# google-research/sparf

Hardware: NVIDIA H100
Metric: rays/sec (fwd+bwd, 128 samples/ray) (higher is better)
Workload: dtype fp32 in / out; GEMMs on Hopper wgmma with a 3-pass error-compensated split (fp16 halves forward, bf16 halves backward), fp32 accumulation; fp32 CUDA cores for encoding / activations / compositing

## Files before the change

### sparf_b200/csrc/gemm_wgmma.cu

```cuda
#include <cuda_bf16.h>
#include <cudaTypedefs.h>
#include <cuda_fp16.h>

#include <algorithm>
#include <type_traits>

#include "gemm_wgmma.cuh"

namespace sparf {
namespace {

constexpr int TM = 128, TN = 128, TK = 32;
constexpr int TILE_ELEMS = TM * TK;

struct __align__(128) WgSmem {
  uint16_t a[2][TILE_ELEMS];
  uint16_t b[2][TILE_ELEMS];
};

__device__ __forceinline__ int sw_off(int r, int k) { return (((r >> 3) * (TK / 8) + (k >> 3)) << 6) + ((r & 7) << 3) + (k & 7); }

__device__ __forceinline__ uint64_t smem_desc(const void* p) {
  uint32_t a = static_cast<uint32_t>(__cvta_generic_to_shared(p));
  uint64_t d = (uint64_t)((a & 0x3FFFF) >> 4);
// ... 777 lines not shown
      mbar_wait(&empty[s], ((it / NST) & 1) ^ 1);
      uint8_t* st = smem + s * STAGE_BYTES;
      if (x.div == 1) {
        if (lane == 0) {
          mbar_expect_tx(&full[s], abytes + TK * TM * 4);
          bulk_g2s(st, a.tile(by, kt0 + j), abytes, &full[s]);
          tensor_g2s(st + 2 * TILE_BYTES, xmap, k0, m0, &full[s]);
        }
        continue;
      }
      if (lane == 0) {
        mbar_expect_tx(&full[s], abytes + min(TK, x.M - m0) * rbytes);
        bulk_g2s(st, a.tile(by, kt0 + j), abytes, &full[s]);
      }
      __syncwarp();
      const int m = m0 + lane;
      if (m < x.M) bulk_g2s(st + 2 * TILE_BYTES + lane * (TM * 4), x.X + (size_t)(m / x.div) * x.ldx + k0, rbytes, &full[s]);
    }
  }
}

template <int PASSES, int NST = STAGES>
__device__ __forceinline__ void convert_staged(const Staged& x, const Units& w, uint64_t* full, uint64_t* conv) {
  extern __shared__ __align__(1024) uint8_t smem[];
  const int t = threadIdx.x - CONSUMERS, lane = t & 31;
  int it = 0;
  for (int u = blockIdx.x; u < w.tiles * w.nsplit; u += gridDim.x) {
    int bx, by, kt0, nk;
    w.get(u, bx, by, kt0, nk);
    const bool kin = bx * TM + t < x.K, bits = x.bits && by == 0;
    const int bword = bx * (TM / 32) + (t >> 5);
    for (int j = 0; j < nk; ++j, ++it) {
      const int s = it % NST, m0 = (kt0 + j) * TK;
      mbar_wait(&full[s], (it / NST) & 1);
      uint8_t* st = smem + s * STAGE_BYTES + 2 * TILE_BYTES;
      const float* src = reinterpret_cast<const float*>(st);
      float v[TK];
      if (kin && m0 + TK <= x.M) {
#pragma unroll
        for (int r = 0; r < TK; ++r) v[r] = src[r * TM + t];
      } else {
#pragma unroll
        for (int r = 0; r < TK; ++r) v[r] = kin && m0 + r < x.M ? src[r * TM + t] : 0.f;
      }
      if (bits) {
        uint32_t word = 0;
#pragma unroll
        for (int r = 0; r < TK; ++r) {
          const uint32_t b = __ballot_sync(0xffffffffu, v[r] > 0.f);
          if (lane == r) word = b;
        }
        if (m0 + lane < x.M && bword < x.kw) x.bits[(size_t)(m0 + lane) * x.kw + bword] = word;
      }
      converter_sync();
      uint16_t* img = reinterpret_cast<uint16_t*>(st);
#pragma unroll
      for (int o = 0; o < TK / 8; ++o) {
        float e8[8];
#pragma unroll
        for (int e = 0; e < 8; ++e) e8[e] = v[8 * o + e];
        uint4 hi, lo;
        split8_mul(e8, hi, lo);
        const int off = sw_off(t, 8 * o);
        *reinterpret_cast<uint4*>(img + off) = hi;
        if (PASSES == 3) *reinterpret_cast<uint4*>(img + TILE_ELEMS + off) = lo;
      }
      fence_proxy_async();
      __syncwarp();
      if (lane == 0) mbar_arrive(&conv[s]);
    }
  }
}

__device__ __forceinline__ int part_off(int r, int c) { return r * TN + (((c >> 3) ^ (r & 7)) << 3) + (c & 7); }

__device__ __forceinline__ void presum_epilogue(const float (&acc)[64], float* part, bool first, bool flush, int bx, int by,
                                                const Epi& e) {
  const int lane = threadIdx.x & 31, w = threadIdx.x >> 5;
#pragma unroll
  for (int i = 0; i < 64; i += 2) {
    float2* p = reinterpret_cast<float2*>(part + part_off(frag_row(i), frag_col(i)));
    if (first) {
      *p = make_float2(acc[i], acc[i + 1]);
    } else {
      const float2 o = *p;
      *p = make_float2(o.x + acc[i], o.y + acc[i + 1]);
    }
  }
  if (!flush) return;
  __syncwarp();
  const int m0 = by * TM, n0 = bx * TN;
  float* out = e.out + e.col_off + n0;
  for (int i = 0; i < 16; ++i) {
    const int r = 16 * w + i, m = m0 + r;
    if (m >= e.M) continue;
#pragma unroll
    for (int q = 0; q < TN / 32; ++q) {
      const int c = 32 * q + lane, n = n0 + c;
      if (n < e.N && n < e.Kv) atomicAdd(out + (size_t)m * e.ldo + c, part[part_off(r, c)]);
    }
  }
  __syncwarp();
}

template <int PASSES, bool DYN = false>
__global__ void __launch_bounds__(STAGED_THREADS, 1) wg_gemm_staged_kernel(Opnd a, Staged x, Units w, Epi e, RowCount rc,
                                                                           int ctas, const __grid_constant__ CUtensorMap xmap) {
  extern __shared__ __align__(1024) uint8_t smem[];
  if constexpr (DYN) {
    x.M = (int)live_rows<true, false>(x.M, rc);
    if (x.M == 0) return;
    w.nk = (x.M + TK - 1) / TK;
    w.nsplit = max(1, min(w.nk, (ctas + w.tiles - 1) / w.tiles * ((w.nk + 1023) / 1024)));
  }
  float* part = reinterpret_cast<float*>(smem + STAGED_STAGES * STAGE_BYTES);
  uint64_t* full = reinterpret_cast<uint64_t*>(smem + STAGED_STAGES * STAGE_BYTES + PART_BYTES);
  uint64_t* empty = full + STAGED_STAGES;
  uint64_t* conv = empty + STAGED_STAGES;
  if (threadIdx.x == 0) {
    for (int i = 0; i < STAGED_STAGES; ++i) {
      mbar_init(&full[i], 1);
      mbar_init(&empty[i], CONSUMERS / 32);
      mbar_init(&conv[i], 4);
    }
    asm volatile("fence.mbarrier_init.release.cluster;\n" ::: "memory");
  }
  __syncthreads();
  if (threadIdx.x >= CONSUMERS + 128) {
    asm volatile("setmaxnreg.dec.sync.aligned.u32 40;\n" ::: "memory");
    if (threadIdx.x < CONSUMERS + 128 + 32) produce_staged<PASSES, STAGED_STAGES>(a, x, &xmap, w, full, empty);
    return;
  }
  if (threadIdx.x >= CONSUMERS) {
    asm volatile("setmaxnreg.dec.sync.aligned.u32 64;\n" ::: "memory");
    convert_staged<PASSES, STAGED_STAGES>(x, w, full, conv);
    return;
  }
  asm volatile("setmaxnreg.inc.sync.aligned.u32 200;\n" ::: "memory");
  const int units = w.tiles * w.nsplit, grid = gridDim.x;
  int it = 0;
  for (int u = blockIdx.x; u < units; u += grid) {
    int bx, by, kt0, nk;
    w.get(u, bx, by, kt0, nk);
    float acc[64];
    mma_unit<false, PASSES, true, STAGED_STAGES>(acc, nk, it, full, empty, conv);
    const int t = u % w.tiles;
    const bool first = u < grid || (u - grid) % w.tiles != t;
    const bool flush = u + grid >= units || (u + grid) % w.tiles != t;
    presum_epilogue(acc, part, first, flush, bx, by, e);
  }
}

constexpr int CH_W = 256;
constexpr int CH_M = 64;
constexpr int CH_KS = CH_W / TK;
constexpr int CH_ENC_KS = 2;
constexpr int CH_HALF = CH_M * TK * 2;
constexpr int CH_STAGES = 4;
constexpr int CH_ENC = CH_KS * 2 * CH_HALF;
constexpr int CH_RING = CH_ENC + CH_ENC_KS * 2 * CH_HALF;
constexpr int CH_BAR = CH_RING + CH_STAGES * STAGE_BYTES;
constexpr int CH_SMEM = CH_BAR + (2 * CH_STAGES + 2) * 8;

struct Chain {
  int M, nl, skip, enc_ks;
  const uint16_t* enc;
  const uint16_t* w[SPARF_MAX_TRUNK];
  const float* bias[SPARF_MAX_TRUNK];
  float* H[SPARF_MAX_TRUNK];
  uint16_t* last;
  uint32_t* bits[SPARF_MAX_TRUNK];
};

__host__ __device__ __forceinline__ int chain_ks(int l, int skip, int enc_ks) {
  return l == 0 ? enc_ks : CH_KS + (l == skip ? enc_ks : 0);
}

template <int PASSES>
__device__ __forceinline__ void chain_produce(const Chain& c, int M, int tiles, uint64_t* full, uint64_t* empty, uint64_t* enc_full,
                                              uint64_t* enc_empty) {
  extern __shared__ __align__(1024) uint8_t smem[];
  constexpr int HB = PASSES == 3 ? 2 : 1;
  int it = 0, n = 0;
  for (int t = blockIdx.x; t < tiles; t += gridDim.x) {
    if (t * CH_M >= M) continue;
    mbar_wait(enc_empty, (n & 1) ^ 1);
    ++n;
    mbar_expect_tx(enc_full, c.enc_ks * HB * CH_HALF);
    for (int kt = 0; kt < c.enc_ks; ++kt)
      for (int h = 0; h < HB; ++h)
        bulk_g2s(smem + CH_ENC + (kt * 2 + h) * CH_HALF,
                 c.enc + (((size_t)(t >> 1) * c.enc_ks + kt) * 2 + h) * TILE_ELEMS + (t & 1) * (CH_M * TK), CH_HALF, enc_full);
    for (int l = 0; l < c.nl; ++l) {
      const int nk = chain_ks(l, c.skip, c.enc_ks);
      for (int kt = 0; kt < nk; ++kt, ++it) {
        const int s = it % CH_STAGES;
        mbar_wait(&empty[s], ((it / CH_STAGES) & 1) ^ 1);
        uint8_t* st = smem + CH_RING + s * STAGE_BYTES;
        mbar_expect_tx(&full[s], 2 * HB * TILE_BYTES);
        for (int g = 0; g < 2; ++g)
          bulk_g2s(st + g * 2 * TILE_BYTES, c.w[l] + ((size_t)g * nk + kt) * 2 * TILE_ELEMS, HB * TILE_BYTES, &full[s]);
      }
    }
  }
}

template <bool F16, int PASSES>
__device__ __forceinline__ void chain_mma(float (&acc)[64], int nk, int na, int& it, uint64_t* full, uint64_t* empty) {
  extern __shared__ __align__(1024) uint8_t smem[];
  const int wg = threadIdx.x >> 7, lane = threadIdx.x & 31;
  float acc_lo[PASSES == 3 ? 64 : 1];
#pragma unroll
  for (int i = 0; i < 64; ++i) acc[i] = 0.f;
#pragma unroll
  for (int i = 0; i < (PASSES == 3 ? 64 : 1); ++i) acc_lo[i] = 0.f;
  for (int j = 0; j < nk; ++j, ++it) {
    const int s = it % CH_STAGES;
    mbar_wait(&full[s], (it / CH_STAGES) & 1);
    const uint8_t* a = j < na ? smem + j * 2 * CH_HALF : smem + CH_ENC + (j - na) * 2 * CH_HALF;
    const uint8_t* b = smem + CH_RING + s * STAGE_BYTES + wg * 2 * TILE_BYTES;
    wgmma_fence();
#pragma unroll
    for (int ks = 0; ks < TK / 16; ++ks) {
      const uint64_t ahi = smem_desc(a + ks * 256), bhi = smem_desc(b + ks * 256);
      if constexpr (PASSES == 3) {
        wgmma_m64n128k16<F16>(acc_lo, smem_desc(a + CH_HALF + ks * 256), bhi);
        wgmma_m64n128k16<F16>(acc_lo, ahi, smem_desc(b + TILE_BYTES + ks * 256));
      }
      wgmma_m64n128k16<F16>(acc, ahi, bhi);
    }
    wgmma_commit();
    wgmma_wait_1();
    if (j > 0 && lane == 0) mbar_arrive(&empty[(it + CH_STAGES - 1) % CH_STAGES]);
  }
  wgmma_wait_all();
  if (lane == 0) mbar_arrive(&empty[(it + CH_STAGES - 1) % CH_STAGES]);
  if constexpr (PASSES == 3) {
#pragma unroll
    for (int i = 0; i < 64; ++i) acc[i] += ldexpf(acc_lo[i], -LO_SHIFT);
  }
}

template <bool F16, int PASSES>
__device__ __forceinline__ void chain_epilogue(float (&acc)[64], const Chain& c, int M, int l, int t) {
  extern __shared__ __align__(1024) uint8_t smem[];
  const int wg = threadIdx.x >> 7, wq = (threadIdx.x >> 5) & 3, lane = threadIdx.x & 31;
  const float* bias = c.bias[l];
#pragma unroll
  for (int i = 0; i < 64; i += 2) {
    const int m = t * CH_M + wq * 16 + (lane >> 2) + ((i >> 1) & 1) * 8, n = wg * TN + (i >> 2) * 8 + (lane & 3) * 2;
    if (m >= M) {
      acc[i] = acc[i + 1] = 0.f;
      continue;
    }
    acc[i] = fmaxf(acc[i] + bias[n], 0.f);
    acc[i + 1] = fmaxf(acc[i + 1] + bias[n + 1], 0.f);
  }
  const bool last = l == c.nl - 1;
  if (last && !c.last) return;
  uint16_t* img = last ? c.last + (size_t)(t >> 1) * CH_KS * 2 * TILE_ELEMS + (t & 1) * (CH_M * TK)
                       : reinterpret_cast<uint16_t*>(smem);
  const int kstride = last ? 2 * TILE_ELEMS : CH_HALF, lo_off = last ? TILE_ELEMS : CH_HALF / 2;
#pragma unroll
  for (int j = 0; j < 16; ++j) {
    uint16_t* kt = img + (size_t)(4 * wg + (j >> 2)) * kstride;
#pragma unroll
    for (int h = 0; h < 2; ++h) {
      uint32_t hi, lo;
      split2<F16>(acc[4 * j + 2 * h], acc[4 * j + 2 * h + 1], hi, lo);
      const int core = (2 * wq + h) * (TK / 8) + (j & 3);
      reinterpret_cast<uint32_t*>(kt + core * 64)[lane] = hi;
      if (PASSES == 3) reinterpret_cast<uint32_t*>(kt + lo_off + core * 64)[lane] = lo;
    }
  }
}

__device__ __forceinline__ void chain_store(const float (&acc)[64], float* H, int M, int t) {
  const int wg = threadIdx.x >> 7, wq = (threadIdx.x >> 5) & 3, lane = threadIdx.x & 31;
#pragma unroll
  for (int i = 0; i < 64; i += 2) {
    const int m = t * CH_M + wq * 16 + (lane >> 2) + ((i >> 1) & 1) * 8, n = wg * TN + (i >> 2) * 8 + (lane & 3) * 2;
    if (m < M) *reinterpret_cast<float2*>(H + (size_t)m * CH_W + n) = make_float2(acc[i], acc[i + 1]);
  }
}

__device__ __forceinline__ void chain_store_bits(const float (&acc)[64], uint32_t* bits, int M, int t) {
  const int wg = threadIdx.x >> 7, wq = (threadIdx.x >> 5) & 3, lane = threadIdx.x & 31;
#pragma unroll
  for (int h = 0; h < 2; ++h) {
    uint32_t mine = 0;
#pragma unroll
    for (int q = 0; q < 4; ++q) {
      uint32_t w = 0;
#pragma unroll
      for (int jj = 0; jj < 4; ++jj) {
        const int i = 4 * (4 * q + jj) + 2 * h, b = 8 * jj + 2 * (lane & 3);
        w |= (uint32_t)(acc[i] > 0.f) << b | (uint32_t)(acc[i + 1] > 0.f) << (b + 1);
      }
      w |= __shfl_xor_sync(0xffffffffu, w, 1);
      w |= __shfl_xor_sync(0xffffffffu, w, 2);
      if ((lane & 3) == q) mine = w;
    }
    const int m = t * CH_M + wq * 16 + (lane >> 2) + 8 * h;
    if (m < M) bits[(size_t)m * (CH_W / 32) + wg * 4 + (lane & 3)] = mine;
  }
}

template <bool F16, int PASSES, bool DYN = false, bool BITS = false, bool SPAN = false>
__global__ void __launch_bounds__(GEMM_THREADS, 1) trunk_chain_kernel(const Chain c, RowCount rc) {
  extern __shared__ __align__(1024) uint8_t smem[];
  const int M = (int)live_rows<DYN, SPAN>(c.M, rc);
  if (DYN && M == 0) return;
  const int tiles = (M + TM - 1) / TM * 2;
  uint64_t* full = reinterpret_cast<uint64_t*>(smem + CH_BAR);
  uint64_t* empty = full + CH_STAGES;
  uint64_t* enc_full = empty + CH_STAGES;
  uint64_t* enc_empty = enc_full + 1;
  if (threadIdx.x == 0) {
    for (int i = 0; i < CH_STAGES; ++i) {
      mbar_init(&full[i], 1);
      mbar_init(&empty[i], CONSUMERS / 32);
    }
    mbar_init(enc_full, 1);
    mbar_init(enc_empty, CONSUMERS / 32);
    asm volatile("fence.mbarrier_init.release.cluster;\n" ::: "memory");
  }
  __syncthreads();
  if (threadIdx.x >= CONSUMERS) {
    asm volatile("setmaxnreg.dec.sync.aligned.u32 40;\n" ::: "memory");
    if (threadIdx.x == CONSUMERS) chain_produce<PASSES>(c, M, tiles, full, empty, enc_full, enc_empty);
    return;
  }
  asm volatile("setmaxnreg.inc.sync.aligned.u32 232;\n" ::: "memory");
  const int enc_last = c.skip > 0 && c.skip < c.nl ? c.skip : 0;
  const long long s0 = row_start<SPAN>(rc);
  int it = 0, n = 0;
  for (int t = blockIdx.x; t < tiles; t += gridDim.x) {
    if (t * CH_M >= M) {
      if (c.last)
        for (int i = 0; i < CH_KS * (PASSES == 3 ? 2 : 1); ++i)
          reinterpret_cast<uint4*>(c.last + ((size_t)(t >> 1) * CH_KS * 2 + (PASSES == 3 ? i : 2 * i)) * TILE_ELEMS +
                                   (t & 1) * (CH_M * TK))[threadIdx.x] = make_uint4(0, 0, 0, 0);
      continue;
    }
    mbar_wait(enc_full, n & 1);
    ++n;
    for (int l = 0; l < c.nl; ++l) {
      float acc[64];
      chain_mma<F16, PASSES>(acc, chain_ks(l, c.skip, c.enc_ks), l == 0 ? 0 : CH_KS, it, full, empty);
      if (l == enc_last && (threadIdx.x & 31) == 0) mbar_arrive(enc_empty);
      consumer_sync();
      chain_epilogue<F16, PASSES>(acc, c, M, l, t);
      if (l + 1 < c.nl) {
        fence_proxy_async();
        consumer_sync();
      }
      if (c.H[l]) chain_store(acc, c.H[l] + s0 * CH_W, M, t);
      if (BITS && c.bits[l]) chain_store_bits(acc, c.bits[l] + s0 * (CH_W / 32), M, t);
    }
  }
}

template <bool F16, int PASSES>
static int launch_chain(const Chain& c, int ctas, RowCount rc, cudaStream_t st) {
  bool bits = false;
  for (int l = 0; l < c.nl; ++l) bits |= c.bits[l] != nullptr;
  auto kernel = bits ? (rc.rows ? trunk_chain_kernel<F16, PASSES, true, true> : trunk_chain_kernel<F16, PASSES, false, true>)
                     : (rc.rows ? trunk_chain_kernel<F16, PASSES, true> : trunk_chain_kernel<F16, PASSES>);
  if (rc.start) {
    if (!bits) {
      set_error("trunk_chain: a row start needs the mask bits (taped forward)");
      return SPARF_ERR_UNSUPPORTED;
    }
    kernel = trunk_chain_kernel<F16, PASSES, true, true, true>;
  }
  SPARF_CHECK_CUDA(cudaFuncSetAttribute(kernel, cudaFuncAttributeMaxDynamicSharedMemorySize, CH_SMEM));
  kernel<<<std::min(2 * ceil_div(c.M, TM), ctas), GEMM_THREADS, CH_SMEM, st>>>(c, rc);
  SPARF_CHECK_LAUNCH("trunk_chain_kernel");
  return SPARF_OK;
}

struct DgChain {
  int M, top, tr_ks;
  const uint16_t* in;
  const uint16_t* w[SPARF_MAX_TRUNK];
  const uint32_t* bits[SPARF_MAX_TRUNK];
  float* db[SPARF_MAX_TRUNK];
  uint16_t* tr[SPARF_MAX_TRUNK];
  uint16_t* row[SPARF_MAX_TRUNK];
};

template <int DP>
__device__ __forceinline__ void dg_produce(const DgChain& c, int M, int tiles, uint64_t* full, uint64_t* empty, uint64_t* act_full,
                                           uint64_t* act_empty) {
  extern __shared__ __align__(1024) uint8_t smem[];
  constexpr int HB = DP == 3 ? 2 : 1;
  int it = 0, n = 0;
  for (int t = blockIdx.x; t < tiles; t += gridDim.x) {
    if (t * CH_M >= M) continue;
    mbar_wait(act_empty, (n & 1) ^ 1);
    ++n;
    mbar_expect_tx(act_full, CH_KS * HB * CH_HALF);
    for (int kt = 0; kt < CH_KS; ++kt)
      for (int h = 0; h < HB; ++h)
        bulk_g2s(smem + (kt * 2 + h) * CH_HALF,
                 c.in + (((size_t)(t >> 1) * CH_KS + kt) * 2 + h) * TILE_ELEMS + (t & 1) * (CH_M * TK), CH_HALF, act_full);
    for (int l = c.top; l >= 1; --l)
      for (int kt = 0; kt < CH_KS; ++kt, ++it) {
        const int s = it % CH_STAGES;
        mbar_wait(&empty[s], ((it / CH_STAGES) & 1) ^ 1);
        uint8_t* st = smem + CH_RING + s * STAGE_BYTES;
        mbar_expect_tx(&full[s], 2 * HB * TILE_BYTES);
        for (int g = 0; g < 2; ++g)
          bulk_g2s(st + g * 2 * TILE_BYTES, c.w[l] + ((size_t)g * CH_KS + kt) * 2 * TILE_ELEMS, HB * TILE_BYTES, &full[s]);
      }
  }
}

__device__ __forceinline__ void dg_mask_words(uint4 (&wd)[2], const uint32_t* bits, int M, int t) {
  const int wg = threadIdx.x >> 7, wq = (threadIdx.x >> 5) & 3, lane = threadIdx.x & 31;
#pragma unroll
  for (int h = 0; h < 2; ++h) {
    const int m = t * CH_M + wq * 16 + (lane >> 2) + 8 * h;
    wd[h] = m < M ? *reinterpret_cast<const uint4*>(bits + (size_t)m * (CH_W / 32) + wg * 4) : make_uint4(0, 0, 0, 0);
  }
}

template <int PASSES>
__device__ __forceinline__ void dg_split(const float (&acc)[64], uint16_t* img, int kstride, int lo_off) {
  const int wg = threadIdx.x >> 7, wq = (threadIdx.x >> 5) & 3, lane = threadIdx.x & 31;
#pragma unroll
  for (int j = 0; j < 16; ++j) {
    uint16_t* kt = img + (size_t)(4 * wg + (j >> 2)) * kstride;
#pragma unroll
    for (int h = 0; h < 2; ++h) {
      uint32_t hi, lo;
      split2<false>(acc[4 * j + 2 * h], acc[4 * j + 2 * h + 1], hi, lo);
      const int core = (2 * wq + h) * (TK / 8) + (j & 3);
      reinterpret_cast<uint32_t*>(kt + core * 64)[lane] = hi;
      if (PASSES == 3) reinterpret_cast<uint32_t*>(kt + lo_off + core * 64)[lane] = lo;
    }
  }
}

template <int DP, int TP>
__device__ __forceinline__ void dg_zero_tile(const DgChain& c, int t) {
  const uint4 z = make_uint4(0, 0, 0, 0);
  for (int l = c.top; l >= 1; --l) {
    if (c.row[l])
      for (int i = 0; i < CH_KS * (DP == 3 ? 2 : 1); ++i)
        reinterpret_cast<uint4*>(c.row[l] + ((size_t)(t >> 1) * CH_KS * 2 + (DP == 3 ? i : 2 * i)) * TILE_ELEMS +
                                 (t & 1) * (CH_M * TK))[threadIdx.x] = z;
    for (int g = 0; g < 2; ++g)
      for (int kt = 2 * t; kt < 2 * t + 2 && kt < c.tr_ks; ++kt)
        for (int h = 0; h < (TP == 3 ? 2 : 1); ++h)
          for (int i = threadIdx.x; i < TILE_ELEMS / 8; i += CONSUMERS)
            reinterpret_cast<uint4*>(c.tr[l] + (((size_t)g * c.tr_ks + kt) * 2 + h) * TILE_ELEMS)[i] = z;
  }
}

template <int DP, int TP, bool DYN = false>
__global__ void __launch_bounds__(GEMM_THREADS, 1) dgrad_chain_kernel(const DgChain c, RowCount rc) {
  extern __shared__ __align__(1024) uint8_t smem[];
  const int M = (int)live_rows<DYN, false>(c.M, rc);
  if (DYN && M == 0) return;
  const int tiles = (M + TM - 1) / TM * 2;
  uint64_t* full = reinterpret_cast<uint64_t*>(smem + CH_BAR);
  uint64_t* empty = full + CH_STAGES;
  uint64_t* act_full = empty + CH_STAGES;
  uint64_t* act_empty = act_full + 1;
  float* red = reinterpret_cast<float*>(smem + CH_ENC);
  if (threadIdx.x == 0) {
    for (int i = 0; i < CH_STAGES; ++i) {
      mbar_init(&full[i], 1);
      mbar_init(&empty[i], CONSUMERS / 32);
    }
    mbar_init(act_full, 1);
    mbar_init(act_empty, CONSUMERS / 32);
    asm volatile("fence.mbarrier_init.release.cluster;\n" ::: "memory");
  }
  __syncthreads();
  if (threadIdx.x >= CONSUMERS) {
    asm volatile("setmaxnreg.dec.sync.aligned.u32 40;\n" ::: "memory");
    if (threadIdx.x == CONSUMERS) dg_produce<DP>(c, M, tiles, full, empty, act_full, act_empty);
    return;
  }
  asm volatile("setmaxnreg.inc.sync.aligned.u32 232;\n" ::: "memory");
  const int wg = threadIdx.x >> 7, wq = (threadIdx.x >> 5) & 3, w = threadIdx.x >> 5, lane = threadIdx.x & 31;
  int it = 0, n = 0;
  for (int t = blockIdx.x; t < tiles; t += gridDim.x) {
    if (t * CH_M >= M) {
      dg_zero_tile<DP, TP>(c, t);
      continue;
    }
    mbar_wait(act_full, n & 1);
    ++n;
    for (int l = c.top; l >= 1; --l) {
      uint4 wd[2];
      dg_mask_words(wd, c.bits[l], M, t);
      float acc[64];
      chain_mma<false, DP>(acc, CH_KS, CH_KS, it, full, empty);
      if (l == 1 && lane == 0) mbar_arrive(act_empty);
      consumer_sync();
      const uint32_t wds[2][4] = {{wd[0].x, wd[0].y, wd[0].z, wd[0].w}, {wd[1].x, wd[1].y, wd[1].z, wd[1].w}};
#pragma unroll
      for (int i = 0; i < 64; i += 2) {
        const int j = i >> 2;
        const uint32_t k = wds[(i >> 1) & 1][j >> 2] >> (8 * (j & 3) + 2 * (lane & 3));
        if (!(k & 1)) acc[i] = 0.f;
        if (!(k & 2)) acc[i + 1] = 0.f;
      }
#pragma unroll
      for (int j = 0; j < 16; ++j)
#pragma unroll
        for (int cc = 0; cc < 2; ++cc) {
          float s = acc[4 * j + cc] + acc[4 * j + 2 + cc];
#pragma unroll
          for (int o = 4; o < 32; o <<= 1) s += __shfl_xor_sync(0xffffffffu, s, o);
          if (lane < 4) red[w * TN + 8 * j + 2 * lane + cc] = s;
        }
      if (l > 1) {
        dg_split<DP>(acc, reinterpret_cast<uint16_t*>(smem), CH_HALF, CH_HALF / 2);
        fence_proxy_async();
      }
      consumer_sync();
      {
        float s = 0.f;
#pragma unroll
        for (int i = 0; i < 4; ++i) s += red[(4 * wg + i) * TN + (threadIdx.x & (TN - 1))];
        atomicAdd(c.db[l] + threadIdx.x, s);
      }
      const int kt = 2 * t + (wq >> 1);
      if (kt < c.tr_ks) {
        uint16_t* tp = c.tr[l] + ((size_t)wg * c.tr_ks + kt) * 2 * TILE_ELEMS;
#pragma unroll
        for (int j = 0; j < 16; ++j)
#pragma unroll
          for (int h = 0; h < 2; ++h) {
            uint32_t hi, lo;
            split2<false>(acc[4 * j + 2 * h], acc[4 * j + 2 * h + 1], hi, lo);
            const int core = j * (TK / 8) + 2 * (wq & 1) + h;
            reinterpret_cast<uint32_t*>(tp + core * 64)[lane] = movmatrix_trans(hi);
            if (TP == 3) reinterpret_cast<uint32_t*>(tp + TILE_ELEMS + core * 64)[lane] = movmatrix_trans(lo);
          }
      }
      if (c.row[l])
        dg_split<DP>(acc, c.row[l] + (size_t)(t >> 1) * CH_KS * 2 * TILE_ELEMS + (t & 1) * (CH_M * TK), 2 * TILE_ELEMS, TILE_ELEMS);
    }
  }
}

template <int DP, int TP>
static int launch_dgrad_chain(const DgChain& c, int ctas, RowCount rc, cudaStream_t st) {
  auto kernel = rc.rows ? dgrad_chain_kernel<DP, TP, true> : dgrad_chain_kernel<DP, TP>;
  SPARF_CHECK_CUDA(cudaFuncSetAttribute(kernel, cudaFuncAttributeMaxDynamicSharedMemorySize, CH_SMEM));
  kernel<<<std::min(2 * ceil_div(c.M, TM), ctas), GEMM_THREADS, CH_SMEM, st>>>(c, rc);
  SPARF_CHECK_LAUNCH("dgrad_chain_kernel");
  return SPARF_OK;
}

template <bool F16, int PASSES, bool KFAST, class F, bool DYN = false>
static int launch_pack(F f, int rtiles, int ksteps, uint16_t* img, cudaStream_t st, RowCount rc = {nullptr, 0}) {
  pack_kernel<F16, PASSES, KFAST, F, DYN><<<dim3(ksteps, rtiles), 256, 0, st>>>(f, ksteps, img, rc);
  SPARF_CHECK_LAUNCH("pack_kernel");
  return SPARF_OK;
}

template <bool F16, int PASSES, bool F32, int ROWP, int TRP>
static int launch_gemm(const Opnd& a, const Opnd& b, const Units& w, int ctas, const Epi& e, RowCount rc, cudaStream_t st) {
  auto kernel = rc.rows ? wg_gemm_kernel<F16, PASSES, F32, ROWP, TRP, true> : wg_gemm_kernel<F16, PASSES, F32, ROWP, TRP>;
  if (rc.start) {
    if constexpr (F32) {
      kernel = wg_gemm_kernel<F16, PASSES, F32, ROWP, TRP, true, true>;
    } else {
      set_error("a GEMM without an fp32 output takes no row start");
      return SPARF_ERR_UNSUPPORTED;
    }
  }
  SPARF_CHECK_CUDA(cudaFuncSetAttribute(kernel, cudaFuncAttributeMaxDynamicSharedMemorySize, GEMM_SMEM));
  kernel<<<std::min(w.tiles * w.nsplit, ctas), GEMM_THREADS, GEMM_SMEM, st>>>(a, b, w, e, rc);
  SPARF_CHECK_LAUNCH("wg_gemm_kernel");
  return SPARF_OK;
}

static int gemm_ctas(const TcPrec& p) { return p.max_ctas > 0 ? std::min(p.max_ctas, num_sms()) : num_sms(); }

static Units gemm_units(int rta, int rtb, int ksteps, bool split_k, int ctas) {
  Units w{rtb, rta * rtb, 1, ksteps};
  if (split_k) w.nsplit = std::max(1, std::min(ksteps, ceil_div(ctas, w.tiles) * ceil_div(ksteps, 1024)));
  return w;
}

template <bool F16, int PASSES, bool BK, class FB>
static int run(const TcPrec& p, const Opnd& a, int a_rows, FB fb, int b_rows, int ksteps, bool split_k, const Epi& e,
               int row_passes, int tr_passes, cudaStream_t st) {
  const int rta = ceil_div(a_rows, TM), rtb = ceil_div(b_rows, TM);
  SPARF_REQUIRE(p.pack_b && (size_t)rtb * ksteps * 2 * TILE_ELEMS <= p.pack_elems,
                "tc gemm: B operand image needs %zu 16-bit elements, have %zu", (size_t)rtb * ksteps * 2 * TILE_ELEMS,
                p.pack_elems);
  SPARF_TRY((launch_pack<F16, PASSES, BK>(fb, rtb, ksteps, p.pack_b, st)));
  const Opnd b{p.pack_b, nullptr, ksteps, 0};
  const int ctas = gemm_ctas(p);
  const Units w = gemm_units(rta, rtb, ksteps, split_k, ctas);
  const bool f32 = e.out != nullptr;
  const RowCount rc = p.rows;
  SPARF_REQUIRE(!rc.rows || !split_k, "tc gemm: a device row count needs the staged weight-gradient GEMM");
  if (f32 && !row_passes && !tr_passes) return launch_gemm<F16, PASSES, true, 0, 0>(a, b, w, ctas, e, rc, st);
  if (f32 && row_passes == PASSES && !tr_passes) return launch_gemm<F16, PASSES, true, PASSES, 0>(a, b, w, ctas, e, rc, st);
  if (!f32 && row_passes == PASSES && tr_passes == 3) return launch_gemm<F16, PASSES, false, PASSES, 3>(a, b, w, ctas, e, rc, st);
  if (!f32 && row_passes == PASSES && tr_passes == 1) return launch_gemm<F16, PASSES, false, PASSES, 1>(a, b, w, ctas, e, rc, st);
  SPARF_REQUIRE(false, "tc gemm: no kernel for fp32 output %d, row image %d passes, transposed image %d passes", (int)f32,
                row_passes, tr_passes);
}

static int staged_tensor_map(const Staged& x, CUtensorMap* map) {
  static PFN_cuTensorMapEncodeTiled_v12000 encode = nullptr;
  if (!encode) {
    void* fn = nullptr;
    cudaDriverEntryPointQueryResult q;
    SPARF_CHECK_CUDA(cudaGetDriverEntryPoint("cuTensorMapEncodeTiled", &fn, cudaEnableDefault, &q));
    SPARF_REQUIRE(fn && q == cudaDriverEntryPointSuccess, "tc_gemm_tn: the driver has no cuTensorMapEncodeTiled");
    encode = reinterpret_cast<PFN_cuTensorMapEncodeTiled_v12000>(fn);
  }
  const cuuint64_t dims[2] = {(cuuint64_t)x.K, (cuuint64_t)x.M}, pitch[1] = {(cuuint64_t)x.ldx * 4};
  const cuuint32_t box[2] = {TM, TK}, step[2] = {1, 1};
  const CUresult r = encode(map, CU_TENSOR_MAP_DATA_TYPE_FLOAT32, 2, const_cast<float*>(x.X), dims, pitch, box, step,
                            CU_TENSOR_MAP_INTERLEAVE_NONE, CU_TENSOR_MAP_SWIZZLE_NONE, CU_TENSOR_MAP_L2_PROMOTION_L2_256B,
                            CU_TENSOR_MAP_FLOAT_OOB_FILL_NONE);
  SPARF_REQUIRE(r == CUDA_SUCCESS, "tc_gemm_tn: cuTensorMapEncodeTiled failed (%d)", (int)r);
  return SPARF_OK;
}

template <int PASSES>
static int run_staged(const TcPrec& p, const Opnd& gt, int N, const Staged& x, int ksteps, const Epi& e, cudaStream_t st) {
  CUtensorMap xmap{};
  if (x.div == 1 && x.M > 0) SPARF_TRY(staged_tensor_map(x, &xmap));
  const int ctas = gemm_ctas(p);
  const Units w = gemm_units(ceil_div(N, TM), ceil_div(x.K, TM), ksteps, true, ctas);
  auto kernel = p.rows.rows ? wg_gemm_staged_kernel<PASSES, true> : wg_gemm_staged_kernel<PASSES>;
  SPARF_CHECK_CUDA(cudaFuncSetAttribute(kernel, cudaFuncAttributeMaxDynamicSharedMemorySize, STAGED_SMEM));
  kernel<<<std::min(w.tiles * w.nsplit, ctas), STAGED_THREADS, STAGED_SMEM, st>>>(gt, x, w, e, p.rows, ctas, xmap);
  SPARF_CHECK_LAUNCH("wg_gemm_staged_kernel");
  return SPARF_OK;
}

static Opnd opnd(const TcImage& x, const TcImage& y = TcImage{}) { return Opnd{x.p, y.p, x.ks, y.ks}; }

static int set_images(Epi& e, const TcOut& o, int M, int N) {
  SPARF_REQUIRE(!e.accumulate || (!o.row_passes && !o.tr_passes), "tc gemm: images of an accumulated output");
  SPARF_REQUIRE(!o.row_passes || (o.row.p && o.row.ks == ceil_div(N, TK)), "tc gemm: row image needs %d k-steps",
                ceil_div(N, TK));
  SPARF_REQUIRE(!o.tr_passes || (o.tr.p && o.tr.ks == ceil_div(M, TK)), "tc gemm: transposed image needs %d k-steps",
                ceil_div(M, TK));
  e.row = o.row.p; e.row_ks = o.row.ks;
  e.tr = o.tr.p; e.tr_ks = o.tr.ks;
  return SPARF_OK;
}

}

#define SPARF_WG_RUN(BK, ...)                                                                   \
  (p.f16 ? (p.passes == 3 ? run<true, 3, BK>(__VA_ARGS__) : run<true, 1, BK>(__VA_ARGS__))       \
         : (p.passes == 3 ? run<false, 3, BK>(__VA_ARGS__) : run<false, 1, BK>(__VA_ARGS__)))
#define SPARF_WG_PACK(KFAST, ...)                                                                                 \
  (p.f16 ? (p.passes == 3 ? launch_pack<true, 3, KFAST>(__VA_ARGS__) : launch_pack<true, 1, KFAST>(__VA_ARGS__)) \
         : (p.passes == 3 ? launch_pack<false, 3, KFAST>(__VA_ARGS__) : launch_pack<false, 1, KFAST>(__VA_ARGS__)))

size_t tc_image_elems(int rows, int cols) { return (size_t)ceil_div(rows, TM) * ceil_div(cols, TK) * 2 * TILE_ELEMS; }

size_t tc_pack_elems(int rows, int ksteps_rows, int cols) {
  return (size_t)ceil_div(std::max(rows, cols), TM) * ksteps_rows * 2 * TILE_ELEMS;
}

int tc_pack_rows(TcPrec p, int M, int K, const float* X, int ldx, int div, TcImage img, cudaStream_t st) {
  SPARF_REQUIRE((p.passes == 1 || p.passes == 3) && img.p && img.ks == ceil_div(K, TK), "tc_pack_rows: passes=%d ks=%d K=%d",
                p.passes, img.ks, K);
  if (p.rows.rows) {
    const Rows f{X, ldx, K, div, M};
    return p.f16 ? (p.passes == 3 ? launch_pack<true, 3, true, Rows, true>(f, ceil_div(M, TM), img.ks, img.p, st, p.rows)
                                  : launch_pack<true, 1, true, Rows, true>(f, ceil_div(M, TM), img.ks, img.p, st, p.rows))
                 : (p.passes == 3 ? launch_pack<false, 3, true, Rows, true>(f, ceil_div(M, TM), img.ks, img.p, st, p.rows)
                                  : launch_pack<false, 1, true, Rows, true>(f, ceil_div(M, TM), img.ks, img.p, st, p.rows));
  }
  return SPARF_WG_PACK(true, Rows{X, ldx, K, div, M}, ceil_div(M, TM), img.ks, img.p, st);
}

int tc_pack_cols(TcPrec p, int M, int N, const float* X, int ldx, TcImage img, cudaStream_t st) {
  SPARF_REQUIRE((p.passes == 1 || p.passes == 3) && img.p && img.ks == ceil_div(M, TK), "tc_pack_cols: passes=%d ks=%d M=%d",
                p.passes, img.ks, M);
  return SPARF_WG_PACK(false, Cols{X, ldx, M, N}, ceil_div(N, TM), img.ks, img.p, st);
}

int tc_gemm_nt(TcPrec p, int act, int M, int N, TcImage a1, int K1v, TcImage a2, int K2v, const float* W, int ldw, int wcol2,
               const float* bias, float* Y, int ldy, const TcOut& out, cudaStream_t st) {
  SPARF_REQUIRE((p.passes == 1 || p.passes == 3) && (act == 0 || act == 1) && Y, "tc_gemm_nt: passes=%d act=%d", p.passes, act);
  const int ks = a1.ks + (a2.p ? a2.ks : 0);
  Epi e{};
  e.kind = 0; e.M = M; e.N = N; e.act = act; e.bias = bias; e.out = Y; e.ldo = ldy;
  e.pairs = N % 2 == 0 && pair_aligned(Y, ldy);
  SPARF_TRY(set_images(e, out, M, N));
  return SPARF_WG_RUN(true, p, opnd(a1, a2.p ? a2 : TcImage{}), M, NtB{W, ldw, wcol2, K1v, K2v, N, a1.ks}, N, ks, false, e,
                      out.row_passes, out.tr_passes, st);
}

bool tc_chain_supported(int W, int E3p, int nt, int skip) {
  return W == CH_W && E3p <= CH_ENC_KS * TK && nt >= 3 && nt <= SPARF_MAX_TRUNK && skip != 0 && skip < nt;
}

int tc_chain_ksteps(int l, int skip, int E3p) { return chain_ks(l, skip, ceil_div(E3p, TK)); }
// ... 425 lines not shown
```

Measured before the change: 246,100.

## Restructure forward trunk chain to 128-row tiles with N-half weight streaming

The forward fused MLP trunk kernel now processes 128-row tiles. Each consumer warpgroup owns 64 rows and both warpgroups share one 128-wide N-half weight stage, looping over the two N halves sequentially. Before, each tile was 64 rows with each warpgroup taking a different N half. The change is meant to halve weight traffic per row and cut the number of tiles. In exchange it adds per-warpgroup encoding barriers, named-barrier syncs, and register staging of the first half's packed activations, which raises register pressure. The dgrad chain keeps its old layout under renamed constants.

```diff
diff --git a/sparf_b200/csrc/gemm_wgmma.cu b/sparf_b200/csrc/gemm_wgmma.cu
--- a/sparf_b200/csrc/gemm_wgmma.cu
+++ b/sparf_b200/csrc/gemm_wgmma.cu
@@ -953,15 +953,20 @@
 }
 
 constexpr int CH_W = 256;
-constexpr int CH_M = 64;
 constexpr int CH_KS = CH_W / TK;
 constexpr int CH_ENC_KS = 2;
-constexpr int CH_HALF = CH_M * TK * 2;
+constexpr int CH_HALF = 64 * TK * 2;
 constexpr int CH_STAGES = 4;
-constexpr int CH_ENC = CH_KS * 2 * CH_HALF;
-constexpr int CH_RING = CH_ENC + CH_ENC_KS * 2 * CH_HALF;
-constexpr int CH_BAR = CH_RING + CH_STAGES * STAGE_BYTES;
-constexpr int CH_SMEM = CH_BAR + (2 * CH_STAGES + 2) * 8;
+constexpr int FW_STAGE_BYTES = 2 * TILE_BYTES;
+constexpr int FW_ENC = CH_KS * 2 * TILE_BYTES;
+constexpr int FW_RING = FW_ENC + CH_ENC_KS * 2 * TILE_BYTES;
+constexpr int FW_BAR = FW_RING + CH_STAGES * FW_STAGE_BYTES;
+constexpr int FW_SMEM = FW_BAR + (2 * CH_STAGES + 4) * 8;
+constexpr int DG_M = 64;
+constexpr int DG_RED = CH_KS * 2 * CH_HALF;
+constexpr int DG_RING = DG_RED + CH_ENC_KS * 2 * CH_HALF;
+constexpr int DG_BAR = DG_RING + CH_STAGES * STAGE_BYTES;
+constexpr int DG_SMEM = DG_BAR + (2 * CH_STAGES + 2) * 8;
 
 struct Chain {
   int M, nl, skip, enc_ks;
@@ -977,31 +982,77 @@
   return l == 0 ? enc_ks : CH_KS + (l == skip ? enc_ks : 0);
 }
 
+template <bool F16, int PASSES>
+__device__ __forceinline__ void dg_mma(float (&acc)[64], int nk, int& it, uint64_t* full, uint64_t* empty) {
+  extern __shared__ __align__(1024) uint8_t smem[];
+  const int wg = threadIdx.x >> 7, lane = threadIdx.x & 31;
+  float acc_lo[PASSES == 3 ? 64 : 1];
+#pragma unroll
+  for (int i = 0; i < 64; ++i) acc[i] = 0.f;
+#pragma unroll
+  for (int i = 0; i < (PASSES == 3 ? 64 : 1); ++i) acc_lo[i] = 0.f;
+  for (int j = 0; j < nk; ++j, ++it) {
+    const int s = it % CH_STAGES;
+    mbar_wait(&full[s], (it / CH_STAGES) & 1);
+    const uint8_t* a = smem + j * 2 * CH_HALF;
+    const uint8_t* b = smem + DG_RING + s * STAGE_BYTES + wg * 2 * TILE_BYTES;
+    wgmma_fence();
+#pragma unroll
+    for (int ks = 0; ks < TK / 16; ++ks) {
+      const uint64_t ahi = smem_desc(a + ks * 256), bhi = smem_desc(b + ks * 256);
+      if constexpr (PASSES == 3) {
+        wgmma_m64n128k16<F16>(acc_lo, smem_desc(a + CH_HALF + ks * 256), bhi);
+        wgmma_m64n128k16<F16>(acc_lo, ahi, smem_desc(b + TILE_BYTES + ks * 256));
+      }
+      wgmma_m64n128k16<F16>(acc, ahi, bhi);
+    }
+    wgmma_commit();
+    wgmma_wait_1();
+    if (j > 0 && lane == 0) mbar_arrive(&empty[(it + CH_STAGES - 1) % CH_STAGES]);
+  }
+  wgmma_wait_all();
+  if (lane == 0) mbar_arrive(&empty[(it + CH_STAGES - 1) % CH_STAGES]);
+  if constexpr (PASSES == 3) {
+#pragma unroll
+    for (int i = 0; i < 64; ++i) acc[i] += ldexpf(acc_lo[i], -LO_SHIFT);
+  }
+}
+
+__device__ __forceinline__ void wg_sync() { asm volatile("bar.sync %0, 128;\n" ::"r"(2 + (threadIdx.x >> 7)) : "memory"); }
+
+template <int HB>
+__device__ __forceinline__ void chain_stage(const uint16_t* src, int it, uint64_t* full, uint64_t* empty) {
+  extern __shared__ __align__(1024) uint8_t smem[];
+  const int s = it % CH_STAGES;
+  mbar_wait(&empty[s], ((it / CH_STAGES) & 1) ^ 1);
+  mbar_expect_tx(&full[s], HB * TILE_BYTES);
+  bulk_g2s(smem + FW_RING + s * FW_STAGE_BYTES, src, HB * TILE_BYTES, &full[s]);
+}
+
+template <int HB>
+__device__ __forceinline__ void chain_rows(uint8_t* dst, const uint16_t* src, int ks, int g, int n, uint64_t* bar_full,
+                                           uint64_t* bar_empty) {
+  mbar_wait(bar_empty, (n & 1) ^ 1);
+  mbar_expect_tx(bar_full, ks * HB * CH_HALF);
+  for (int kt = 0; kt < ks; ++kt)
+    for (int h = 0; h < HB; ++h)
+      bulk_g2s(dst + (kt * 2 + h) * TILE_BYTES + g * CH_HALF, src + (kt * 2 + h) * TILE_ELEMS + g * (64 * TK), CH_HALF,
+               bar_full);
+}
+
 template <int PASSES>
-__device__ __forceinline__ void chain_produce(const Chain& c, int M, int tiles, uint64_t* full, uint64_t* empty, uint64_t* enc_full,
+__device__ __forceinline__ void chain_produce(const Chain& c, int tiles, uint64_t* full, uint64_t* empty, uint64_t* enc_full,
                                               uint64_t* enc_empty) {
   extern __shared__ __align__(1024) uint8_t smem[];
   constexpr int HB = PASSES == 3 ? 2 : 1;
   int it = 0, n = 0;
-  for (int t = blockIdx.x; t < tiles; t += gridDim.x) {
-    if (t * CH_M >= M) continue;
-    mbar_wait(enc_empty, (n & 1) ^ 1);
-    ++n;
-    mbar_expect_tx(enc_full, c.enc_ks * HB * CH_HALF);
-    for (int kt = 0; kt < c.enc_ks; ++kt)
-      for (int h = 0; h < HB; ++h)
-        bulk_g2s(smem + CH_ENC + (kt * 2 + h) * CH_HALF,
-                 c.enc + (((size_t)(t >> 1) * c.enc_ks + kt) * 2 + h) * TILE_ELEMS + (t & 1) * (CH_M * TK), CH_HALF, enc_full);
+  for (int t = blockIdx.x; t < tiles; t += gridDim.x, ++n) {
+    for (int g = 0; g < 2; ++g)
+      chain_rows<HB>(smem + FW_ENC, c.enc + (size_t)t * c.enc_ks * 2 * TILE_ELEMS, c.enc_ks, g, n, &enc_full[g], &enc_empty[g]);
     for (int l = 0; l < c.nl; ++l) {
       const int nk = chain_ks(l, c.skip, c.enc_ks);
-      for (int kt = 0; kt < nk; ++kt, ++it) {
-        const int s = it % CH_STAGES;
-        mbar_wait(&empty[s], ((it / CH_STAGES) & 1) ^ 1);
-        uint8_t* st = smem + CH_RING + s * STAGE_BYTES;
-        mbar_expect_tx(&full[s], 2 * HB * TILE_BYTES);
-        for (int g = 0; g < 2; ++g)
-          bulk_g2s(st + g * 2 * TILE_BYTES, c.w[l] + ((size_t)g * nk + kt) * 2 * TILE_ELEMS, HB * TILE_BYTES, &full[s]);
-      }
+      for (int nh = 0; nh < 2; ++nh)
+        for (int kt = 0; kt < nk; ++kt, ++it) chain_stage<HB>(c.w[l] + ((size_t)nh * nk + kt) * 2 * TILE_ELEMS, it, full, empty);
     }
   }
 }
@@ -1018,14 +1069,14 @@
   for (int j = 0; j < nk; ++j, ++it) {
     const int s = it % CH_STAGES;
     mbar_wait(&full[s], (it / CH_STAGES) & 1);
-    const uint8_t* a = j < na ? smem + j * 2 * CH_HALF : smem + CH_ENC + (j - na) * 2 * CH_HALF;
-    const uint8_t* b = smem + CH_RING + s * STAGE_BYTES + wg * 2 * TILE_BYTES;
+    const uint8_t* a = (j < na ? smem + j * 2 * TILE_BYTES : smem + FW_ENC + (j - na) * 2 * TILE_BYTES) + wg * CH_HALF;
+    const uint8_t* b = smem + FW_RING + s * FW_STAGE_BYTES;
     wgmma_fence();
 #pragma unroll
     for (int ks = 0; ks < TK / 16; ++ks) {
       const uint64_t ahi = smem_desc(a + ks * 256), bhi = smem_desc(b + ks * 256);
       if constexpr (PASSES == 3) {
-        wgmma_m64n128k16<F16>(acc_lo, smem_desc(a + CH_HALF + ks * 256), bhi);
+        wgmma_m64n128k16<F16>(acc_lo, smem_desc(a + TILE_BYTES + ks * 256), bhi);
         wgmma_m64n128k16<F16>(acc_lo, ahi, smem_desc(b + TILE_BYTES + ks * 256));
       }
       wgmma_m64n128k16<F16>(acc, ahi, bhi);
@@ -1043,13 +1094,40 @@
 }
 
 template <bool F16, int PASSES>
-__device__ __forceinline__ void chain_epilogue(float (&acc)[64], const Chain& c, int M, int l, int t) {
-  extern __shared__ __align__(1024) uint8_t smem[];
-  const int wg = threadIdx.x >> 7, wq = (threadIdx.x >> 5) & 3, lane = threadIdx.x & 31;
-  const float* bias = c.bias[l];
+__device__ __forceinline__ void chain_pack(const float (&acc)[64], uint32_t (&hi)[32], uint32_t (&lo)[PASSES == 3 ? 32 : 1]) {
+#pragma unroll
+  for (int p = 0; p < 32; ++p) {
+    uint32_t l;
+    split2<F16>(acc[2 * p], acc[2 * p + 1], hi[p], l);
+    if (PASSES == 3) lo[p % (PASSES == 3 ? 32 : 1)] = l;
+  }
+}
+
+template <int PASSES>
+__device__ __forceinline__ void chain_put(const uint32_t (&hi)[32], const uint32_t (&lo)[PASSES == 3 ? 32 : 1], uint16_t* img,
+                                          int nh) {
+  const int w = threadIdx.x >> 5, lane = threadIdx.x & 31;
+#pragma unroll
+  for (int j = 0; j < 16; ++j)
+#pragma unroll
+    for (int h = 0; h < 2; ++h) {
+      uint16_t* core = img + (size_t)(4 * nh + (j >> 2)) * 2 * TILE_ELEMS + ((2 * w + h) * (TK / 8) + (j & 3)) * 64;
+      reinterpret_cast<uint32_t*>(core)[lane] = hi[2 * j + h];
+      if (PASSES == 3) reinterpret_cast<uint32_t*>(core + TILE_ELEMS)[lane] = lo[(2 * j + h) % (PASSES == 3 ? 32 : 1)];
+    }
+}
+
+template <bool F16, int PASSES>
+__device__ __forceinline__ void chain_split(const float (&acc)[64], uint16_t* img, int nh) {
+  uint32_t hi[32], lo[PASSES == 3 ? 32 : 1];
+  chain_pack<F16, PASSES>(acc, hi, lo);
+  chain_put<PASSES>(hi, lo, img, nh);
+}
+
+__device__ __forceinline__ void chain_values(float (&acc)[64], const float* bias, int M, int t, int nh) {
 #pragma unroll
   for (int i = 0; i < 64; i += 2) {
-    const int m = t * CH_M + wq * 16 + (lane >> 2) + ((i >> 1) & 1) * 8, n = wg * TN + (i >> 2) * 8 + (lane & 3) * 2;
+    const int m = t * TM + frag_row(i), n = nh * TN + frag_col(i);
     if (m >= M) {
       acc[i] = acc[i + 1] = 0.f;
       continue;
@@ -1057,36 +1135,18 @@
     acc[i] = fmaxf(acc[i] + bias[n], 0.f);
     acc[i + 1] = fmaxf(acc[i + 1] + bias[n + 1], 0.f);
   }
-  const bool last = l == c.nl - 1;
-  if (last && !c.last) return;
-  uint16_t* img = last ? c.last + (size_t)(t >> 1) * CH_KS * 2 * TILE_ELEMS + (t & 1) * (CH_M * TK)
-                       : reinterpret_cast<uint16_t*>(smem);
-  const int kstride = last ? 2 * TILE_ELEMS : CH_HALF, lo_off = last ? TILE_ELEMS : CH_HALF / 2;
-#pragma unroll
-  for (int j = 0; j < 16; ++j) {
-    uint16_t* kt = img + (size_t)(4 * wg + (j >> 2)) * kstride;
-#pragma unroll
-    for (int h = 0; h < 2; ++h) {
-      uint32_t hi, lo;
-      split2<F16>(acc[4 * j + 2 * h], acc[4 * j + 2 * h + 1], hi, lo);
-      const int core = (2 * wq + h) * (TK / 8) + (j & 3);
-      reinterpret_cast<uint32_t*>(kt + core * 64)[lane] = hi;
-      if (PASSES == 3) reinterpret_cast<uint32_t*>(kt + lo_off + core * 64)[lane] = lo;
-    }
-  }
-}
-
-__device__ __forceinline__ void chain_store(const float (&acc)[64], float* H, int M, int t) {
-  const int wg = threadIdx.x >> 7, wq = (threadIdx.x >> 5) & 3, lane = threadIdx.x & 31;
+}
+
+__device__ __forceinline__ void chain_store(const float (&acc)[64], float* H, int M, int t, int nh) {
 #pragma unroll
   for (int i = 0; i < 64; i += 2) {
-    const int m = t * CH_M + wq * 16 + (lane >> 2) + ((i >> 1) & 1) * 8, n = wg * TN + (i >> 2) * 8 + (lane & 3) * 2;
+    const int m = t * TM + frag_row(i), n = nh * TN + frag_col(i);
     if (m < M) *reinterpret_cast<float2*>(H + (size_t)m * CH_W + n) = make_float2(acc[i], acc[i + 1]);
   }
 }
 
-__device__ __forceinline__ void chain_store_bits(const float (&acc)[64], uint32_t* bits, int M, int t) {
-  const int wg = threadIdx.x >> 7, wq = (threadIdx.x >> 5) & 3, lane = threadIdx.x & 31;
+__device__ __forceinline__ void chain_store_bits(const float (&acc)[64], uint32_t* bits, int M, int t, int nh) {
+  const int lane = threadIdx.x & 31;
 #pragma unroll
   for (int h = 0; h < 2; ++h) {
     uint32_t mine = 0;
@@ -1102,8 +1162,8 @@
       w |= __shfl_xor_sync(0xffffffffu, w, 2);
       if ((lane & 3) == q) mine = w;
     }
-    const int m = t * CH_M + wq * 16 + (lane >> 2) + 8 * h;
-    if (m < M) bits[(size_t)m * (CH_W / 32) + wg * 4 + (lane & 3)] = mine;
+    const int m = t * TM + frag_row(2 * h);
+    if (m < M) bits[(size_t)m * (CH_W / 32) + nh * 4 + (lane & 3)] = mine;
   }
 }
 
@@ -1112,52 +1172,59 @@
   extern __shared__ __align__(1024) uint8_t smem[];
   const int M = (int)live_rows<DYN, SPAN>(c.M, rc);
   if (DYN && M == 0) return;
-  const int tiles = (M + TM - 1) / TM * 2;
-  uint64_t* full = reinterpret_cast<uint64_t*>(smem + CH_BAR);
+  const int tiles = (M + TM - 1) / TM;
+  uint64_t* full = reinterpret_cast<uint64_t*>(smem + FW_BAR);
   uint64_t* empty = full + CH_STAGES;
   uint64_t* enc_full = empty + CH_STAGES;
-  uint64_t* enc_empty = enc_full + 1;
+  uint64_t* enc_empty = enc_full + 2;
   if (threadIdx.x == 0) {
     for (int i = 0; i < CH_STAGES; ++i) {
       mbar_init(&full[i], 1);
       mbar_init(&empty[i], CONSUMERS / 32);
     }
-    mbar_init(enc_full, 1);
-    mbar_init(enc_empty, CONSUMERS / 32);
+    for (int g = 0; g < 2; ++g) {
+      mbar_init(&enc_full[g], 1);
+      mbar_init(&enc_empty[g], 4);
+    }
     asm volatile("fence.mbarrier_init.release.cluster;\n" ::: "memory");
   }
   __syncthreads();
   if (threadIdx.x >= CONSUMERS) {
     asm volatile("setmaxnreg.dec.sync.aligned.u32 40;\n" ::: "memory");
-    if (threadIdx.x == CONSUMERS) chain_produce<PASSES>(c, M, tiles, full, empty, enc_full, enc_empty);
+    if (threadIdx.x == CONSUMERS) chain_produce<PASSES>(c, tiles, full, empty, enc_full, enc_empty);
     return;
   }
   asm volatile("setmaxnreg.inc.sync.aligned.u32 232;\n" ::: "memory");
+  const int wg = threadIdx.x >> 7, lane = threadIdx.x & 31;
   const int enc_last = c.skip > 0 && c.skip < c.nl ? c.skip : 0;
   const long long s0 = row_start<SPAN>(rc);
   int it = 0, n = 0;
-  for (int t = blockIdx.x; t < tiles; t += gridDim.x) {
-    if (t * CH_M >= M) {
-      if (c.last)
-        for (int i = 0; i < CH_KS * (PASSES == 3 ? 2 : 1); ++i)
-          reinterpret_cast<uint4*>(c.last + ((size_t)(t >> 1) * CH_KS * 2 + (PASSES == 3 ? i : 2 * i)) * TILE_ELEMS +
-                                   (t & 1) * (CH_M * TK))[threadIdx.x] = make_uint4(0, 0, 0, 0);
-      continue;
-    }
-    mbar_wait(enc_full, n & 1);
-    ++n;
+  for (int t = blockIdx.x; t < tiles; t += gridDim.x, ++n) {
+    mbar_wait(&enc_full[wg], n & 1);
     for (int l = 0; l < c.nl; ++l) {
-      float acc[64];
-      chain_mma<F16, PASSES>(acc, chain_ks(l, c.skip, c.enc_ks), l == 0 ? 0 : CH_KS, it, full, empty);
-      if (l == enc_last && (threadIdx.x & 31) == 0) mbar_arrive(enc_empty);
-      consumer_sync();
-      chain_epilogue<F16, PASSES>(acc, c, M, l, t);
-      if (l + 1 < c.nl) {
-        fence_proxy_async();
-        consumer_sync();
-      }
-      if (c.H[l]) chain_store(acc, c.H[l] + s0 * CH_W, M, t);
-      if (BITS && c.bits[l]) chain_store_bits(acc, c.bits[l] + s0 * (CH_W / 32), M, t);
+      const int nk = chain_ks(l, c.skip, c.enc_ks), na = l == 0 ? 0 : CH_KS;
+      const bool last = l == c.nl - 1;
+      uint32_t hi0[32], lo0[PASSES == 3 ? 32 : 1];
+#pragma unroll
+      for (int nh = 0; nh < 2; ++nh) {
+        float acc[64];
+        chain_mma<F16, PASSES>(acc, nk, na, it, full, empty);
+        if (nh == 1 && l == enc_last && lane == 0) mbar_arrive(&enc_empty[wg]);
+        chain_values(acc, c.bias[l], M, t, nh);
+        if (last) {
+          if (c.last) chain_split<F16, PASSES>(acc, c.last + (size_t)t * CH_KS * 2 * TILE_ELEMS, nh);
+        } else if (nh == 0) {
+          chain_pack<F16, PASSES>(acc, hi0, lo0);
+        } else {
+          wg_sync();
+          chain_put<PASSES>(hi0, lo0, reinterpret_cast<uint16_t*>(smem), 0);
+          chain_split<F16, PASSES>(acc, reinterpret_cast<uint16_t*>(smem), 1);
+          fence_proxy_async();
+          wg_sync();
+        }
+        if (c.H[l]) chain_store(acc, c.H[l] + s0 * CH_W, M, t, nh);
+        if (BITS && c.bits[l]) chain_store_bits(acc, c.bits[l] + s0 * (CH_W / 32), M, t, nh);
+      }
     }
   }
 }
@@ -1175,8 +1242,8 @@
     }
     kernel = trunk_chain_kernel<F16, PASSES, true, true, true>;
   }
-  SPARF_CHECK_CUDA(cudaFuncSetAttribute(kernel, cudaFuncAttributeMaxDynamicSharedMemorySize, CH_SMEM));
-  kernel<<<std::min(2 * ceil_div(c.M, TM), ctas), GEMM_THREADS, CH_SMEM, st>>>(c, rc);
+  SPARF_CHECK_CUDA(cudaFuncSetAttribute(kernel, cudaFuncAttributeMaxDynamicSharedMemorySize, FW_SMEM));
+  kernel<<<std::min(ceil_div(c.M, TM), ctas), GEMM_THREADS, FW_SMEM, st>>>(c, rc);
   SPARF_CHECK_LAUNCH("trunk_chain_kernel");
   return SPARF_OK;
 }
@@ -1198,19 +1265,19 @@
   constexpr int HB = DP == 3 ? 2 : 1;
   int it = 0, n = 0;
   for (int t = blockIdx.x; t < tiles; t += gridDim.x) {
-    if (t * CH_M >= M) continue;
+    if (t * DG_M >= M) continue;
     mbar_wait(act_empty, (n & 1) ^ 1);
     ++n;
     mbar_expect_tx(act_full, CH_KS * HB * CH_HALF);
     for (int kt = 0; kt < CH_KS; ++kt)
       for (int h = 0; h < HB; ++h)
         bulk_g2s(smem + (kt * 2 + h) * CH_HALF,
-                 c.in + (((size_t)(t >> 1) * CH_KS + kt) * 2 + h) * TILE_ELEMS + (t & 1) * (CH_M * TK), CH_HALF, act_full);
+                 c.in + (((size_t)(t >> 1) * CH_KS + kt) * 2 + h) * TILE_ELEMS + (t & 1) * (DG_M * TK), CH_HALF, act_full);
     for (int l = c.top; l >= 1; --l)
       for (int kt = 0; kt < CH_KS; ++kt, ++it) {
         const int s = it % CH_STAGES;
         mbar_wait(&empty[s], ((it / CH_STAGES) & 1) ^ 1);
-        uint8_t* st = smem + CH_RING + s * STAGE_BYTES;
+        uint8_t* st = smem + DG_RING + s * STAGE_BYTES;
         mbar_expect_tx(&full[s], 2 * HB * TILE_BYTES);
         for (int g = 0; g < 2; ++g)
           bulk_g2s(st + g * 2 * TILE_BYTES, c.w[l] + ((size_t)g * CH_KS + kt) * 2 * TILE_ELEMS, HB * TILE_BYTES, &full[s]);
@@ -1222,7 +1289,7 @@
   const int wg = threadIdx.x >> 7, wq = (threadIdx.x >> 5) & 3, lane = threadIdx.x & 31;
 #pragma unroll
   for (int h = 0; h < 2; ++h) {
-    const int m = t * CH_M + wq * 16 + (lane >> 2) + 8 * h;
+    const int m = t * DG_M + wq * 16 + (lane >> 2) + 8 * h;
     wd[h] = m < M ? *reinterpret_cast<const uint4*>(bits + (size_t)m * (CH_W / 32) + wg * 4) : make_uint4(0, 0, 0, 0);
   }
 }
@@ -1251,7 +1318,7 @@
     if (c.row[l])
       for (int i = 0; i < CH_KS * (DP == 3 ? 2 : 1); ++i)
         reinterpret_cast<uint4*>(c.row[l] + ((size_t)(t >> 1) * CH_KS * 2 + (DP == 3 ? i : 2 * i)) * TILE_ELEMS +
-                                 (t & 1) * (CH_M * TK))[threadIdx.x] = z;
+                                 (t & 1) * (DG_M * TK))[threadIdx.x] = z;
     for (int g = 0; g < 2; ++g)
       for (int kt = 2 * t; kt < 2 * t + 2 && kt < c.tr_ks; ++kt)
         for (int h = 0; h < (TP == 3 ? 2 : 1); ++h)
@@ -1266,11 +1333,11 @@
   const int M = (int)live_rows<DYN, false>(c.M, rc);
   if (DYN && M == 0) return;
   const int tiles = (M + TM - 1) / TM * 2;
-  uint64_t* full = reinterpret_cast<uint64_t*>(smem + CH_BAR);
+  uint64_t* full = reinterpret_cast<uint64_t*>(smem + DG_BAR);
   uint64_t* empty = full + CH_STAGES;
   uint64_t* act_full = empty + CH_STAGES;
   uint64_t* act_empty = act_full + 1;
-  float* red = reinterpret_cast<float*>(smem + CH_ENC);
+  float* red = reinterpret_cast<float*>(smem + DG_RED);
   if (threadIdx.x == 0) {
     for (int i = 0; i < CH_STAGES; ++i) {
       mbar_init(&full[i], 1);
@@ -1290,7 +1357,7 @@
   const int wg = threadIdx.x >> 7, wq = (threadIdx.x >> 5) & 3, w = threadIdx.x >> 5, lane = threadIdx.x & 31;
   int it = 0, n = 0;
   for (int t = blockIdx.x; t < tiles; t += gridDim.x) {
-    if (t * CH_M >= M) {
+    if (t * DG_M >= M) {
       dg_zero_tile<DP, TP>(c, t);
       continue;
     }
@@ -1300,7 +1367,7 @@
       uint4 wd[2];
       dg_mask_words(wd, c.bits[l], M, t);
       float acc[64];
-      chain_mma<false, DP>(acc, CH_KS, CH_KS, it, full, empty);
+      dg_mma<false, DP>(acc, CH_KS, it, full, empty);
       if (l == 1 && lane == 0) mbar_arrive(act_empty);
       consumer_sync();
       const uint32_t wds[2][4] = {{wd[0].x, wd[0].y, wd[0].z, wd[0].w}, {wd[1].x, wd[1].y, wd[1].z, wd[1].w}};
@@ -1346,7 +1413,7 @@
           }
       }
       if (c.row[l])
-        dg_split<DP>(acc, c.row[l] + (size_t)(t >> 1) * CH_KS * 2 * TILE_ELEMS + (t & 1) * (CH_M * TK), 2 * TILE_ELEMS, TILE_ELEMS);
+        dg_split<DP>(acc, c.row[l] + (size_t)(t >> 1) * CH_KS * 2 * TILE_ELEMS + (t & 1) * (DG_M * TK), 2 * TILE_ELEMS, TILE_ELEMS);
     }
   }
 }
@@ -1354,8 +1421,8 @@
 template <int DP, int TP>
 static int launch_dgrad_chain(const DgChain& c, int ctas, RowCount rc, cudaStream_t st) {
   auto kernel = rc.rows ? dgrad_chain_kernel<DP, TP, true> : dgrad_chain_kernel<DP, TP>;
-  SPARF_CHECK_CUDA(cudaFuncSetAttribute(kernel, cudaFuncAttributeMaxDynamicSharedMemorySize, CH_SMEM));
-  kernel<<<std::min(2 * ceil_div(c.M, TM), ctas), GEMM_THREADS, CH_SMEM, st>>>(c, rc);
+  SPARF_CHECK_CUDA(cudaFuncSetAttribute(kernel, cudaFuncAttributeMaxDynamicSharedMemorySize, DG_SMEM));
+  kernel<<<std::min(2 * ceil_div(c.M, TM), ctas), GEMM_THREADS, DG_SMEM, st>>>(c, rc);
   SPARF_CHECK_LAUNCH("dgrad_chain_kernel");
   return SPARF_OK;
 }
```

Result: faster. 249,300, median of 6 (+1.3%).
